# Tangshitao/Semi-supervised-Adaptive-Distillation

Hardware: AMD Instinct MI355X
Metric: images/sec (student+teacher fwd + student bwd) R50-FPN distill, 1/2/4/8 MI355X (higher is better)
Workload: dtype f32

## Files before the change

include/ssad_kernels.h:

```cpp
#ifndef SSAD_KERNELS_H_
#define SSAD_KERNELS_H_

#include <stddef.h>
#include <stdint.h>

#ifdef __cplusplus
extern "C" {
#endif

#define SSAD_API __attribute__((visibility("default")))

#define SSAD_E_BADARG (-1)
#define SSAD_E_WORKSPACE (-2)
#define SSAD_MAX_LEVELS 8
#define SSAD_MAX_CONV_PROBLEMS 24
#define SSAD_MAX_POWSUM_INPUTS 8

typedef void* ssad_stream_t;


typedef struct {
  float gamma;
  float alpha;
  float beta;
// ... 128 lines not shown
  const float* x;
  float* y;
  const float* aux;
  int N, H, W;
  const float* packed;
  const float* bias;
} ssad_conv_level;

SSAD_API size_t ssad_conv_packed_filter_floats(int M, int K);

SSAD_API int ssad_conv_pack_filter(
    const float* w, int Cout, int Cin, float* packed_fwd, float* packed_dgrad,
    ssad_stream_t stream);

#define SSAD_CONV_RELU 1
#define SSAD_CONV_MASK_AUX 2
#define SSAD_CONV_SIGMOID 4
#define SSAD_CONV_SPLIT_TAIL 8

SSAD_API int ssad_conv3x3_forward(
    const ssad_conv_level* levels_host, int n_levels, const float* packed,
    const float* bias, int Cout, int Cin, int flags, ssad_stream_t stream);

SSAD_API size_t ssad_conv_wino_filter_floats(int M, int K);
SSAD_API int ssad_conv_wino_pack_filter(
    const float* w, int Cout, int Cin, float* packed_fwd, float* packed_dgrad,
    ssad_stream_t stream);
SSAD_API int ssad_conv3x3_forward_wino(
    const ssad_conv_level* levels_host, int n_levels, const float* packed,
    const float* bias, int Cout, int Cin, int flags, ssad_stream_t stream);
SSAD_API int ssad_conv3x3_forward_wino_launches(const ssad_conv_level* levels_host, int n_levels);
SSAD_API int ssad_conv3x3_forward_wino_launches_for(const ssad_conv_level* levels_host, int n_levels, int Cout,
                                                    int Cin, int flags);
SSAD_API int ssad_conv_wino_split_tail(int on);
#define SSAD_MAX_PACK_ENTRIES 32
typedef struct ssad_pack_entry {
  const float* w;
  int Cout, Cin;
  float* packed_fwd;
  float* packed_dgrad;
} ssad_pack_entry;
SSAD_API int ssad_conv_wino_pack_filters(const ssad_pack_entry* entries_host, int n_entries,
                                         ssad_stream_t stream);

SSAD_API size_t ssad_conv_wino24_filter_floats(int M, int K);
SSAD_API int ssad_conv_wino24_pack_filters(const ssad_pack_entry* entries_host, int n_entries, ssad_stream_t stream);
SSAD_API int ssad_conv3x3_forward_wino24(
    const ssad_conv_level* levels_host, int n_levels, const float* packed,
    const float* bias, int Cout, int Cin, int flags, ssad_stream_t stream);

SSAD_API size_t ssad_conv_split_filter_floats(int M, int K);
SSAD_API int ssad_conv_split_pack_filters(const ssad_pack_entry* entries_host, int n_entries, ssad_stream_t stream);
SSAD_API size_t ssad_conv3x3_split_workspace_bytes(const ssad_conv_level* levels_host, int n_levels, int Cin);
SSAD_API int ssad_conv3x3_forward_split(
    const ssad_conv_level* levels_host, int n_levels, const float* packed,
    const float* bias, int Cout, int Cin, int flags, void* workspace, size_t workspace_bytes,
    const unsigned* amax_in, unsigned* amax_out, ssad_stream_t stream);

SSAD_API size_t ssad_conv3x3_wgrad_workspace_bytes(
    const ssad_conv_level* levels_host, int n_levels, int Cout, int Cin);

SSAD_API int ssad_conv3x3_wgrad(
    const ssad_conv_level* levels_host, int n_levels, float* dW, float* db,
    int Cout, int Cin, int accumulate, void* workspace, size_t workspace_bytes,
    ssad_stream_t stream);

SSAD_API size_t ssad_conv3x3_wgrad_split_workspace_bytes(
    const ssad_conv_level* levels_host, int n_levels, int Cout, int Cin);
SSAD_API int ssad_conv3x3_wgrad_split(
    const ssad_conv_level* levels_host, int n_levels, float* dW, float* db,
    int Cout, int Cin, int accumulate, void* workspace, size_t workspace_bytes,
    ssad_stream_t stream);
SSAD_API int ssad_conv3x3_wgrad_split_amax(
    const ssad_conv_level* levels_host, int n_levels, float* dW, float* db,
    int Cout, int Cin, int accumulate, void* workspace, size_t workspace_bytes,
    const unsigned* x_amax, const unsigned* dy_amax, ssad_stream_t stream);

SSAD_API int ssad_split_absmax_levels(const ssad_conv_level* levels_host, int n, int channels, int field,
                                      unsigned* words, ssad_stream_t stream);
SSAD_API int ssad_split_absmax(const float* x, long long n, unsigned* word, ssad_stream_t stream);


SSAD_API size_t ssad_retinanet_anchor_labels_workspace_bytes(
    int levels, int A, int k_min, const int* field_sizes_host, int N, int Gmax);
SSAD_API int ssad_retinanet_anchor_labels(
    const double* cell_anchors, int levels, int A, int k_min, const int* field_sizes_host,
    const int* crop_h_host, const int* crop_w_host, const float* gt_boxes,
    const int* gt_classes, const int* gt_counts, int N, int Gmax, int num_classes,
    float positive_overlap, float negative_overlap, int* const* labels_out_host,
    float* const* locs_out_host, float* const* targets_out_host, int capacity,
    int* counts_out, float* fg_bg_out, void* workspace, size_t workspace_bytes,
    ssad_stream_t stream);


#define SSAD_IMAGE_BLOBS_MAX_BATCH 64
typedef struct ssad_image_norm {
  float div, mean[3], std[3];
  float* out;
} ssad_image_norm;
SSAD_API size_t ssad_image_blobs_workspace_bytes(int N, int Hb, int Wb);
SSAD_API int ssad_image_blobs(
    const unsigned char* src, size_t src_bytes, const long long* offset_host, const int* h_host,
    const int* w_host, const int* out_h_host, const int* out_w_host, const double* scale_host,
    const int* flipped_host, int N, int Hb, int Wb, const ssad_image_norm* norms_host, int n_norms,
    void* workspace, size_t workspace_bytes, ssad_stream_t stream);

// ... 278 lines not shown
```

semi-supervised-adaptive-distillation_amd/csrc/kernels/conv3x3_split.hip:

```cpp
#include <hip/hip_fp16.h>
#include <hip/hip_runtime.h>
#include <stdint.h>
#include <stdlib.h>

#include "conv_internal.h"
#include "ssad_kernels.h"

#include "split_common.h"

namespace {

using namespace ssad_split;

constexpr int TS = 16;
constexpr int HS = TS + 2;
constexpr int CBC = 2;
constexpr int SLOTS = CBC * HS * HS;
constexpr int NLD = 3;
constexpr int STAGE = 4 * NLD * 64;
constexpr int AD = 9;
constexpr int NBUF = 3;
constexpr int MT = 128;
constexpr int HDR = 16;
static_assert(AD == 9 && NLD == 3, "the counted waits below are written for these");

#ifndef SPLIT_ABLATE
#define SPLIT_ABLATE 0
#endif

#ifdef SPLIT_TIMELINE
__device__ unsigned long long g_split_dbg[64][8];
#define SDBG(itn, k) if (dbg_on && (itn) < 64) g_split_dbg[itn][k] = __builtin_readcyclecounter()
#else
#define SDBG(itn, k)
#endif

__host__ __device__ constexpr int cdiv(int a, int b) { return (a + b - 1) / b; }

struct FPackTable {
  ssad_pack_entry e[SSAD_MAX_PACK_ENTRIES];
};
__global__ void split_filter_zero_kernel(const FPackTable t) {
  const ssad_pack_entry& e = t.e[blockIdx.x];
  if (threadIdx.x < HDR) {
    if (e.packed_fwd) reinterpret_cast<unsigned*>(e.packed_fwd)[threadIdx.x] = 0u;
    if (e.packed_dgrad) reinterpret_cast<unsigned*>(e.packed_dgrad)[threadIdx.x] = 0u;
  }
}
__global__ __launch_bounds__(kThreads) void split_filter_amax_kernel(const FPackTable t) {
  const ssad_pack_entry& e = t.e[blockIdx.y];
  const long long n = (long long)e.Cout * e.Cin * 9;
  unsigned m = 0;
  for (long long i = (long long)blockIdx.x * kThreads + threadIdx.x; i < n; i += (long long)gridDim.x * kThreads) {
    const unsigned a = __float_as_uint(e.w[i]) & 0x7fffffffu;
    m = m > a ? m : a;
  }
  __shared__ unsigned red[kThreads / 64];
#pragma unroll
  for (int o = 32; o > 0; o >>= 1) {
    const unsigned other = (unsigned)__shfl_xor((int)m, o, 64);
    m = m > other ? m : other;
  }
  if ((threadIdx.x & 63) == 0) red[threadIdx.x >> 6] = m;
  __syncthreads();
  if (threadIdx.x == 0) {
    unsigned r = red[0];
    for (int w = 1; w < kThreads / 64; ++w) r = r > red[w] ? r : red[w];
    if (r) {
      if (e.packed_fwd) atomicMax(reinterpret_cast<unsigned*>(e.packed_fwd), r);
      if (e.packed_dgrad) atomicMax(reinterpret_cast<unsigned*>(e.packed_dgrad), r);
    }
  }
}
__global__ __launch_bounds__(kThreads) void split_filter_pack_kernel(const FPackTable t) {
  const ssad_pack_entry& e = t.e[blockIdx.y];
  const bool dg = blockIdx.z == 1;
  float* dst = dg ? e.packed_dgrad : e.packed_fwd;
  if (!dst) return;
  const int M = dg ? e.Cin : e.Cout, K = dg ? e.Cout : e.Cin;
  const int KB = (K + 7) >> 3;
  const long long slots = 9LL * KB * M;
  const float s = pow2f(15 - split_exponent(reinterpret_cast<const unsigned*>(dst)[0]));
  uint4* out = reinterpret_cast<uint4*>(dst + HDR);
  for (long long i = (long long)blockIdx.x * kThreads + threadIdx.x; i < slots; i += (long long)gridDim.x * kThreads) {
    const int m = (int)(i % M), kb = (int)((i / M) % KB), tap = (int)(i / ((long long)M * KB));
    float v[8];
#pragma unroll
    for (int j = 0; j < 8; ++j) {
      const int k = kb * 8 + j;
      v[j] = k >= K ? 0.0f : dg ? e.w[((long long)k * e.Cin + m) * 9 + (8 - tap)] : e.w[((long long)m * e.Cin + k) * 9 + tap];
    }
    half8 hi, lo;
    split8(v, s, hi, lo);
    out[i] = __builtin_bit_cast(uint4, hi);
    out[slots + i] = __builtin_bit_cast(uint4, lo);
  }
}

struct SLevels {
  const uint4* x[kMaxLv];
  float* y[kMaxLv];
  const float* aux[kMaxLv];
  const float* w[kMaxLv];
  const float* bias[kMaxLv];
  int N[kMaxLv], H[kMaxLv], W[kMaxLv];
  int tile0[kMaxLv + 1];
  const unsigned* amax;
  unsigned* amax_out;
  int n_levels, C, M, relu, sigmoid, mblocks, items;
};

template <bool MASKED>
__global__ __launch_bounds__(kThreads, 1) void conv3x3_split_kernel(const SLevels q) {
  __shared__ uint4 lds[NBUF * 2 * STAGE];
  __shared__ unsigned wg_max[kThreads / 64];
  const int tid = threadIdx.x, lane = tid & 63;
  const int wave = __builtin_amdgcn_readfirstlane(tid >> 6);
  const int wo = wave & 1, wp = wave >> 1;
  const int j = lane & 31, h = lane >> 5;
  const int C = q.C, M = q.M;
  const int CB = (C + 7) >> 3;
  const int nchunks = (CB + CBC - 1) / CBC;
  const unsigned w_lo_off = (unsigned)(9LL * CB * M * 16);
  const unsigned lds_base = (unsigned)(uintptr_t)(lds_ptr)lds;
  const int brow = wp * 8 + (j >> 4), bcol = (j & 16) ? ((j - 2) & 15) : j;
  const int bbase = (h * HS + brow) * HS + bcol;

  struct Item {
    int lv, n, y0, x0, ocb, H, W, N;
  };
  auto decode = [&](int it) {
    Item o;
    const int xcd = it & 7, seq = it >> 3;
    const int mb = seq % q.mblocks;
    int t = (seq / q.mblocks) * 8 + xcd;
    int lv = 0;
    for (int l = 1; l < q.n_levels; ++l)
      if (t >= q.tile0[l]) lv = l;
    o.lv = t < q.tile0[q.n_levels] ? lv : -1;
    o.N = q.N[lv]; o.H = q.H[lv]; o.W = q.W[lv];
    const int tiles_x = (o.W + TS - 1) / TS, tiles_y = (o.H + TS - 1) / TS;
    t -= q.tile0[lv];
    const int tx = t % tiles_x; t /= tiles_x;
    const int ty = t % tiles_y;
    o.n = t / tiles_y;
    o.y0 = ty * TS; o.x0 = tx * TS;
    o.ocb = mb * MT;
    return o;
  };
  ssad_dev::rsrc_words xrs = ssad_dev::uniform_rsrc_words(q.x[0], 0), wrs = xrs;
  unsigned dvo[NLD], avo[2], x_lo_off = 0;
  int dcb[NLD], plane16 = 0;
  auto bind = [&](const Item& I) {
    const long long plane = (long long)I.H * I.W;
    plane16 = (int)plane * 16;
    x_lo_off = (unsigned)((long long)I.N * CB * plane16);
    xrs = ssad_dev::uniform_rsrc_words(q.x[I.lv], 2u * x_lo_off);
    wrs = ssad_dev::uniform_rsrc_words(q.w[I.lv] + HDR, 2u * w_lo_off);
#pragma unroll
    for (int i = 0; i < NLD; ++i) {
      const int s = 64 * (wave + 4 * i) + lane;
      const int cbl = s / (HS * HS), r = s % (HS * HS);
      const int gy = I.y0 - 1 + r / HS, gx = I.x0 - 1 + r % HS;
      const bool ok = s < SLOTS && gy >= 0 && gy < I.H && gx >= 0 && gx < I.W;
      dcb[i] = cbl;
      dvo[i] = ok ? (unsigned)((((long long)I.n * CB + cbl) * plane + (long long)gy * I.W + gx) * 16) : kOob;
    }
#pragma unroll
    for (int i = 0; i < 2; ++i) {
      const int oc = I.ocb + wo * 64 + i * 32 + j;
      avo[i] = (unsigned)(h * M + (oc < M ? oc : M - 1)) * 16u;
    }
  };
  auto dma_piece = [&](int chunk, int buf, int i, bool real) {
    const unsigned vo = (real && !(SPLIT_ABLATE & 1) && chunk * CBC + dcb[i] < CB) ? dvo[i] : kOob;
    const int soff = __builtin_amdgcn_readfirstlane(real ? chunk * CBC * plane16 : 0);
    const unsigned dst = lds_base + (unsigned)((buf * 2 * STAGE + 64 * (wave + 4 * i)) * 16);
    dma16(xrs, dst, vo, soff);
    dma16(xrs, dst + STAGE * 16, vo, soff + (int)x_lo_off);
  };
  f32x4 ar[AD][4];
  auto ring_load1 = [&](f32x4& dst, int chunk, int tap, int k, bool real) {
    const int soff = __builtin_amdgcn_readfirstlane(real ? ((tap * CB + chunk * CBC) * M) * 16 + (k >> 1) * (int)w_lo_off : 0);
    const unsigned vo = (real && !(SPLIT_ABLATE & 2)) ? avo[k & 1] : kOob;
    asm volatile("s_nop 4\n\tbuffer_load_dwordx4 %0, %1, %2, %3 offen" : "=v"(dst) : "v"(vo), "s"(wrs), "s"(soff));
  };
  auto ring_load = [&](f32x4 (&dst)[4], int chunk, int tap, bool real) {
#pragma unroll
    for (int k = 0; k < 4; ++k) ring_load1(dst[k], chunk, tap, k, real);
  };
  auto ring_landed = [&]() {
    asm volatile("s_waitcnt vmcnt(0)" ::: "memory");
#pragma unroll
    for (int a = 0; a < AD; ++a) asm volatile("" : "+v"(ar[a][0]), "+v"(ar[a][1]), "+v"(ar[a][2]), "+v"(ar[a][3]));
  };
  int gbuf = 0;
  auto prologue = [&]() {
    int b1 = gbuf + 1; if (b1 >= NBUF) b1 -= NBUF;
#pragma unroll
    for (int i = 0; i < NLD; ++i) dma_piece(0, gbuf, i, true);
#pragma unroll
    for (int i = 0; i < NLD; ++i) dma_piece(1, b1, i, nchunks > 1);
#pragma unroll
    for (int a = 0; a < AD; ++a) ring_load(ar[a], 0, a, true);
  };

  const int G = (int)gridDim.x;
  int it = (int)blockIdx.x;
  Item cur = decode(it);
  while (it < q.items && cur.lv < 0) { it += G; if (it < q.items) cur = decode(it); }
  if (it >= q.items) return;
  bind(cur);
  prologue();
  ring_landed();
  __builtin_amdgcn_s_barrier();

#ifdef SPLIT_TIMELINE
  const bool dbg_on = blockIdx.x == 5 && tid == 0;
  int itn = 0;
#endif
  while (true) {
    SDBG(itn, 0);
    float16v acc[2][4];
    {
      float zero;
      asm volatile("v_mov_b32 %0, 0" : "=v"(zero));
#pragma unroll
      for (int i = 0; i < 2; ++i)
#pragma unroll
        for (int tt = 0; tt < 4; ++tt)
#pragma unroll
          for (int r = 0; r < 16; ++r) acc[i][tt][r] = zero;
    }

    int buf = gbuf;
    for (int c = 0; c < nchunks; ++c) {
      const bool more = c + 1 < nchunks, more2 = c + 2 < nchunks;
      int buf2 = buf + 2; if (buf2 >= NBUF) buf2 -= NBUF;
      const uint4* tile_hi = lds + buf * 2 * STAGE;
      const uint4* tile_lo = tile_hi + STAGE;
      half8 bh[4], bl[4];
      auto read_b = [&](const uint4* tile, int tap, half8 (&bb)[4]) {
        const int dy = tap / 3, dx = tap % 3;
#pragma unroll
        for (int tt = 0; tt < 4; ++tt) bb[tt] = __builtin_bit_cast(half8, tile[bbase + (2 * tt + dy) * HS + dx]);
      };
      read_b(tile_hi, 0, bh);
      read_b(tile_lo, 0, bl);
#pragma unroll
      for (int tap = 0; tap < 9; ++tap) {
        f32x4 (&a)[4] = ar[tap];
        switch (tap) {
          case 0: asm volatile("s_waitcnt vmcnt(38)" : "+v"(a[0]), "+v"(a[1]), "+v"(a[2]), "+v"(a[3])); break;
          case 7: case 8: asm volatile("s_waitcnt vmcnt(34)" : "+v"(a[0]), "+v"(a[1]), "+v"(a[2]), "+v"(a[3])); break;
          default: asm volatile("s_waitcnt vmcnt(36)" : "+v"(a[0]), "+v"(a[1]), "+v"(a[2]), "+v"(a[3])); break;
        }
        const half8 ah0 = __builtin_bit_cast(half8, a[0]), ah1 = __builtin_bit_cast(half8, a[1]);
        const half8 al0 = __builtin_bit_cast(half8, a[2]), al1 = __builtin_bit_cast(half8, a[3]);
        __builtin_amdgcn_sched_barrier(0);
#pragma unroll
        for (int tt = 0; tt < 4; ++tt) {
          acc[0][tt] = __builtin_amdgcn_mfma_f32_32x32x16_f16(ah0, bh[tt], acc[0][tt], 0, 0, 0);
          acc[1][tt] = __builtin_amdgcn_mfma_f32_32x32x16_f16(ah1, bh[tt], acc[1][tt], 0, 0, 0);
          if (tap >= 1) {
            __builtin_amdgcn_sched_barrier(0);
            if (tt < 2) ring_load1(ar[tap - 1][tt], c + 1, tap - 1, tt, more);
            if (tt == 2 && tap - 1 >= 9 - NLD) dma_piece(c + 2, buf2, tap - 1 - (9 - NLD), more2);
            __builtin_amdgcn_sched_barrier(0);
          }
        }
        __builtin_amdgcn_sched_barrier(0);
        if (!(SPLIT_ABLATE & 4)) {
#pragma unroll
          for (int tt = 0; tt < 4; ++tt) {
            acc[0][tt] = __builtin_amdgcn_mfma_f32_32x32x16_f16(al0, bh[tt], acc[0][tt], 0, 0, 0);
            acc[1][tt] = __builtin_amdgcn_mfma_f32_32x32x16_f16(al1, bh[tt], acc[1][tt], 0, 0, 0);
          }
        }
        __builtin_amdgcn_sched_barrier(0);
        if (tap + 1 < 9) read_b(tile_hi, tap + 1, bh);
        __builtin_amdgcn_sched_barrier(0);
#pragma unroll
        for (int tt = 0; tt < 4; ++tt) {
          if (!(SPLIT_ABLATE & 4)) {
            acc[0][tt] = __builtin_amdgcn_mfma_f32_32x32x16_f16(ah0, bl[tt], acc[0][tt], 0, 0, 0);
            acc[1][tt] = __builtin_amdgcn_mfma_f32_32x32x16_f16(ah1, bl[tt], acc[1][tt], 0, 0, 0);
          }
          __builtin_amdgcn_sched_barrier(0);
          if (tt < 2) ring_load1(a[2 + tt], c + 1, tap, 2 + tt, more);
          __builtin_amdgcn_sched_barrier(0);
        }
        if (tap + 1 < 9) read_b(tile_lo, tap + 1, bl);
        if (tap == 8) {
          ring_load1(a[0], c + 1, 8, 0, more);
          ring_load1(a[1], c + 1, 8, 1, more);
          dma_piece(c + 2, buf2, NLD - 1, more2);
        }
        __builtin_amdgcn_sched_barrier(0);
      }
      asm volatile("s_waitcnt vmcnt(42) lgkmcnt(0)" ::: "memory");
      __builtin_amdgcn_s_barrier();
      if (++buf == NBUF) buf = 0;
    }
    SDBG(itn, 1);
    gbuf = buf;
    ring_landed();

    const Item done = cur;
    int nit = it + G;
    Item nxt = done;
    while (nit < q.items) { nxt = decode(nit); if (nxt.lv >= 0) break; nit += G; }
    const bool have_next = nit < q.items;
    const long long plane = (long long)done.H * done.W;
    const int oc_w = done.ocb + wo * 64;
    unsigned pvo[4];
#pragma unroll
    for (int tt = 0; tt < 4; ++tt) {
      const int gy = done.y0 + wp * 8 + 2 * tt + (j >> 4), gx = done.x0 + bcol;
      const bool okp = gy < done.H && gx < done.W;
      const long long pix = (long long)gy * done.W + gx;
      pvo[tt] = okp ? (unsigned)((((long long)done.n * M + 4 * h) * plane + pix) * 4) : kOob;
    }
    SDBG(itn, 2);
#if !(SPLIT_ABLATE & 32)
    if (have_next) {
      bind(nxt);
      prologue();
    }
#endif
    SDBG(itn, 3);

    {
      const int lv = done.lv;
      const int e2 = split_exponent(q.amax[lv]) + split_exponent(reinterpret_cast<const unsigned*>(q.w[lv])[0]) - 30;
      const bool one_scale = e2 >= -126 && e2 <= 127;
      const float sc1 = one_scale ? pow2f(e2) : pow2f(split_exponent(q.amax[lv]) - 15);
      const float sc2 = one_scale ? 1.0f : pow2f(split_exponent(reinterpret_cast<const unsigned*>(q.w[lv])[0]) - 15);
      const unsigned ybytes = (unsigned)((long long)done.N * M * plane * 4);
      const __amdgpu_buffer_rsrc_t yrs = uniform_rsrc(q.y[lv], ybytes);
      const __amdgpu_buffer_rsrc_t mrs = uniform_rsrc(MASKED ? (const void*)q.aux[lv] : (const void*)q.y[lv], ybytes);
      const float* bias = q.bias[lv];
      const __amdgpu_buffer_rsrc_t brs = uniform_rsrc(bias ? (const void*)bias : (const void*)q.y[lv],
                                                      bias ? (unsigned)M * 4u : 0u);
      const bool relu = q.relu, sigm = q.sigmoid;
      const bool ragged = (M & 7) != 0;
      const bool want_max = q.amax_out != nullptr;
      const int plane4 = (int)plane * 4;
      unsigned vmax = 0;
#pragma unroll
      for (int i = 0; i < 2; ++i) {
        const int oc0 = oc_w + i * 32;
        float4 bq[4];
#pragma unroll
        for (int g = 0; g < 4; ++g)
          bq[g] = __builtin_bit_cast(float4, __builtin_amdgcn_raw_buffer_load_b128(brs, (unsigned)h * 16u, (oc0 + 8 * g) * 4, 0));
#pragma unroll
        for (int tt = 0; tt < 4; ++tt) {
          float mk[16];
          if (MASKED) {
#pragma unroll
            for (int r = 0; r < 16; ++r) {
              const int ch = oc0 + 8 * (r >> 2) + (r & 3);
              const unsigned vo = (!ragged || ch + 4 * h < M) ? pvo[tt] : kOob;
              mk[r] = __builtin_bit_cast(float, __builtin_amdgcn_raw_buffer_load_b32(mrs, vo, ch * plane4, 0));
            }
          }
#pragma unroll
          for (int g = 0; g < 4; ++g) {
            if (oc0 + 8 * g >= M) continue;
#pragma unroll
            for (int e = 0; e < 4; ++e) {
              float v = one_scale ? fmaf(acc[i][tt][4 * g + e], sc1, bq[g][e]) : acc[i][tt][4 * g + e] * sc1 * sc2 + bq[g][e];
              if (relu) v = fmaxf(v, 0.0f);
              if (sigm) v = 1.0f / (1.0f + expf(-v));
              if (MASKED) v = mk[4 * g + e] > 0.0f ? v : 0.0f;
              const unsigned vo = (!ragged || oc0 + 8 * g + 4 * h + e < M) ? pvo[tt] : kOob;
              if (want_max) {
                const unsigned av = __float_as_uint(v) & 0x7fffffffu;
                vmax = (vo != kOob && av > vmax) ? av : vmax;
              }
              __builtin_amdgcn_raw_buffer_store_b32(__builtin_bit_cast(unsigned, v), yrs, vo, (oc0 + 8 * g + e) * plane4, 0);
            }
          }
        }
      }
      if (q.amax_out) {
#pragma unroll
        for (int o = 32; o > 0; o >>= 1) {
          const unsigned other = (unsigned)__shfl_xor((int)vmax, o, 64);
          vmax = vmax > other ? vmax : other;
        }
        if (lane == 0) wg_max[wave] = vmax;
      }
    }
#if SPLIT_ABLATE & 32
    if (have_next) {
      asm volatile("s_waitcnt vmcnt(0)" ::: "memory");
      bind(nxt);
      prologue();
    }
#endif
    if (!have_next) {
      if (q.amax_out) {
        __builtin_amdgcn_s_barrier();
        if (tid == 0) {
          unsigned m = wg_max[0];
          for (int w = 1; w < kThreads / 64; ++w) m = m > wg_max[w] ? m : wg_max[w];
          if (m) atomicMax(q.amax_out + done.lv, m);
        }
      }
      asm volatile("s_waitcnt vmcnt(0)" ::: "memory");
      return;
    }
    SDBG(itn, 4);
    ring_landed();
    SDBG(itn, 5);
    __builtin_amdgcn_s_barrier();
    SDBG(itn, 6);
#ifdef SPLIT_TIMELINE
    ++itn;
#endif
    if (q.amax_out && tid == 0) {
      unsigned m = wg_max[0];
      for (int w = 1; w < kThreads / 64; ++w) m = m > wg_max[w] ? m : wg_max[w];
      if (m) atomicMax(q.amax_out + done.lv, m);
    }
    it = nit;
    cur = nxt;
  }
}

struct Plan {
  size_t amax_bytes, total_bytes;
  size_t plane_off[kMaxLv];
  long long slots[kMaxLv];
};
int make_plan(const ssad_conv_level* lv, int n_levels, int Cin, Plan* p) {
  if (!lv || n_levels < 1 || n_levels > kMaxLv || Cin <= 0) return SSAD_E_BADARG;
  const int CB = (Cin + 7) >> 3;
  p->amax_bytes = 256;
  size_t off = p->amax_bytes;
  for (int l = 0; l < n_levels; ++l) {
    if (lv[l].N < 0 || lv[l].H < 0 || lv[l].W < 0) return SSAD_E_BADARG;
    const long long slots = (long long)lv[l].N * CB * lv[l].H * lv[l].W;
    if (slots * 32 >= (1LL << 32)) return SSAD_E_BADARG;
    p->slots[l] = slots;
    p->plane_off[l] = off;
    off += (size_t)slots * 32;
    off = (off + 255) & ~(size_t)255;
  }
  p->total_bytes = off;
  return 0;
}

}

#ifdef SPLIT_TIMELINE
extern "C" __attribute__((visibility("default"))) int ssad_split_dbg_read(void* host) {
  return (int)hipMemcpyFromSymbol(host, HIP_SYMBOL(g_split_dbg), sizeof(g_split_dbg));
}
#endif

extern "C" {

size_t ssad_conv_split_filter_floats(int M, int K) {
  return (size_t)HDR + 2 * (size_t)9 * ((K + 7) >> 3) * M * 4 + 64;
}

int ssad_conv_split_pack_filters(const ssad_pack_entry* entries_host, int n_entries, ssad_stream_t stream) {
  if (n_entries < 0 || (n_entries > 0 && !entries_host)) return SSAD_E_BADARG;
  for (int base = 0; base < n_entries; base += SSAD_MAX_PACK_ENTRIES) {
    const int cnt = n_entries - base < SSAD_MAX_PACK_ENTRIES ? n_entries - base : SSAD_MAX_PACK_ENTRIES;
    FPackTable t;
    long long smax = 0;
    bool any_dgrad = false;
    for (int i = 0; i < cnt; ++i) {
      const ssad_pack_entry& e = entries_host[base + i];
      if (e.Cout <= 0 || e.Cin <= 0 || !e.w || (!e.packed_fwd && !e.packed_dgrad)) return SSAD_E_BADARG;
      t.e[i] = e;
      const long long sf = 9LL * ((e.Cin + 7) >> 3) * e.Cout, sd = 9LL * ((e.Cout + 7) >> 3) * e.Cin;
      smax = sf > smax ? sf : smax;
      if (e.packed_dgrad) { smax = sd > smax ? sd : smax; any_dgrad = true; }
    }
    for (int i = cnt; i < SSAD_MAX_PACK_ENTRIES; ++i) t.e[i] = ssad_pack_entry{};
    hipLaunchKernelGGL(split_filter_zero_kernel, dim3((unsigned)cnt), dim3(64), 0, (hipStream_t)stream, t);
    hipLaunchKernelGGL(split_filter_amax_kernel, dim3(64u, (unsigned)cnt), dim3(kThreads), 0, (hipStream_t)stream, t);
    long long bx = (smax + kThreads - 1) / kThreads;
    if (bx > 512) bx = 512;
    hipLaunchKernelGGL(split_filter_pack_kernel, dim3((unsigned)bx, (unsigned)cnt, any_dgrad ? 2u : 1u), dim3(kThreads), 0,
                       (hipStream_t)stream, t);
  }
  return (int)hipGetLastError();
}

size_t ssad_conv3x3_split_workspace_bytes(const ssad_conv_level* lv, int n_levels, int Cin) {
  Plan p;
  if (make_plan(lv, n_levels, Cin, &p)) return 0;
  return p.total_bytes;
}

int ssad_conv3x3_forward_split(const ssad_conv_level* lv, int n_levels, const float* packed, const float* bias,
                               int Cout, int Cin, int flags, void* workspace, size_t workspace_bytes,
                               const unsigned* amax_in, unsigned* amax_out, ssad_stream_t stream_) {
  hipStream_t stream = (hipStream_t)stream_;
  Plan p;
  const int rc = make_plan(lv, n_levels, Cin, &p);
  if (rc) return rc;
  if (Cout <= 0) return SSAD_E_BADARG;
  if ((flags & SSAD_CONV_MASK_AUX) && (flags & SSAD_CONV_SIGMOID)) return SSAD_E_BADARG;
  if (!workspace || workspace_bytes < p.total_bytes) return SSAD_E_WORKSPACE;
  AmaxTable at;
  ActTable pt;
  SLevels q;
  at.count = pt.count = 0;
  at.amax = (unsigned*)workspace;
  pt.amax = q.amax = (const unsigned*)workspace;
  q.amax_out = amax_out;
  pt.C = Cin;
  int nl = 0, ablocks = 0, pblocks = 0, tiles = 0;
  for (int l = 0; l < n_levels; ++l) {
    const float* pk = lv[l].packed ? lv[l].packed : packed;
    if (!pk) return SSAD_E_BADARG;
    if ((flags & SSAD_CONV_MASK_AUX) && !lv[l].aux) return SSAD_E_BADARG;
    const long long px = (long long)lv[l].N * lv[l].H * lv[l].W;
    if (px * (Cin > Cout ? Cin : Cout) >= (1LL << 29)) return SSAD_E_BADARG;
    if (px == 0) continue;
    const long long n = px * Cin;
    at.x[nl] = pt.x[nl] = lv[l].x;
    at.n[nl] = n;
    at.block_start[nl] = ablocks;
    long long nb = (n / 4 + kThreads * 32 - 1) / (kThreads * 32);
    ablocks += (int)(nb < 1 ? 1 : nb > 512 ? 512 : nb);
    pt.planes[nl] = (uint4*)((char*)workspace + p.plane_off[l]);
    pt.N[nl] = lv[l].N;
    pt.plane[nl] = (long long)lv[l].H * lv[l].W;
    pt.block_start[nl] = pblocks;
    int same = -1;
    for (int j = 0; j < nl && same < 0; ++j)
      if (at.x[j] == lv[l].x && q.N[j] == lv[l].N && q.H[j] == lv[l].H && q.W[j] == lv[l].W) same = j;
    if (same >= 0) pt.planes[nl] = (uint4*)q.x[same];
    else pblocks += (int)((p.slots[l] + kThreads - 1) / kThreads);
    q.x[nl] = (const uint4*)pt.planes[nl];
    q.y[nl] = lv[l].y;
    q.aux[nl] = lv[l].aux;
    q.w[nl] = pk;
    q.bias[nl] = lv[l].packed ? lv[l].bias : bias;
    q.N[nl] = lv[l].N; q.H[nl] = lv[l].H; q.W[nl] = lv[l].W;
    q.tile0[nl] = tiles;
    tiles += lv[l].N * cdiv(lv[l].H, TS) * cdiv(lv[l].W, TS);
    ++nl;
  }
  if (nl == 0) return 0;
  at.block_start[nl] = ablocks;
  pt.block_start[nl] = pblocks;
  q.tile0[nl] = tiles;
  at.count = pt.count = q.n_levels = nl;
  for (int l = nl; l < kMaxLv; ++l) {
    at.x[l] = pt.x[l] = nullptr; at.n[l] = 0; pt.planes[l] = nullptr; pt.N[l] = 0; pt.plane[l] = 0;
    q.x[l] = nullptr; q.y[l] = nullptr; q.aux[l] = nullptr; q.w[l] = nullptr; q.bias[l] = nullptr;
    q.N[l] = q.H[l] = q.W[l] = 0;
    if (l > nl) { at.block_start[l] = ablocks; pt.block_start[l] = pblocks; q.tile0[l] = tiles; }
  }
  q.C = Cin; q.M = Cout;
  q.relu = (flags & SSAD_CONV_RELU) ? 1 : 0;
  q.sigmoid = (flags & SSAD_CONV_SIGMOID) ? 1 : 0;
  q.mblocks = cdiv(Cout, MT);
  if ((amax_in || amax_out) && nl != n_levels) return SSAD_E_BADARG;
  if (amax_in) {
    pt.amax = q.amax = amax_in;
  } else {
    (void)hipMemsetAsync(workspace, 0, p.amax_bytes, stream);
    hipLaunchKernelGGL(split_absmax_kernel, dim3((unsigned)ablocks), dim3(kThreads), 0, stream, at);
  }
  hipLaunchKernelGGL(split_pack_act_kernel, dim3((unsigned)pblocks), dim3(kThreads), 0, stream, pt);
  q.items = cdiv(tiles, 8) * 8 * q.mblocks;
  const int cus = ssad_cu_count();
  const unsigned grid = (unsigned)(q.items < cus ? q.items : cus);
  if (flags & SSAD_CONV_MASK_AUX)
    hipLaunchKernelGGL((conv3x3_split_kernel<true>), dim3(grid), dim3(kThreads), 0, stream, q);
  else
    hipLaunchKernelGGL((conv3x3_split_kernel<false>), dim3(grid), dim3(kThreads), 0, stream, q);
  return (int)hipGetLastError();
}

int ssad_split_absmax_levels(const ssad_conv_level* lv, int n, int channels, int field, unsigned* words,
                             ssad_stream_t stream_) {
  if (!lv || !words || n < 1 || n > kMaxLv || channels <= 0) return SSAD_E_BADARG;
  AmaxTable at;
  int blocks = 0;
  for (int l = 0; l < kMaxLv; ++l) {
    at.x[l] = nullptr; at.n[l] = 0; at.block_start[l] = blocks;
    if (l >= n) continue;
    const long long cnt = (long long)lv[l].N * lv[l].H * lv[l].W * channels;
    at.x[l] = field ? lv[l].aux : lv[l].x;
    at.n[l] = cnt;
    if (cnt && !at.x[l]) return SSAD_E_BADARG;
    long long nb = (cnt / 4 + kThreads * 32 - 1) / (kThreads * 32);
    blocks += (int)(nb < 1 ? 1 : nb > 512 ? 512 : nb);
  }
  at.block_start[kMaxLv] = blocks;
  at.count = n;
  at.amax = words;
  hipLaunchKernelGGL(split_absmax_kernel, dim3((unsigned)blocks), dim3(kThreads), 0, (hipStream_t)stream_, at);
  return (int)hipGetLastError();
}

}
```

semi-supervised-adaptive-distillation_amd/kernels.py:

```python
import ctypes as C
import os

import torch

_HERE = os.path.dirname(os.path.abspath(__file__))
LIB_NAME = "libcaffe2_detectron_ops_hip.so"
LIB_PATH = os.path.join(_HERE, LIB_NAME)

MAX_LEVELS = 8
CONV_RELU = 1
CONV_MASK_AUX = 2
CONV_SIGMOID = 4
CONV_SPLIT_TAIL = 8


class KernelError(RuntimeError):
    pass


class DistillParams(C.Structure):
    _fields_ = [("gamma", C.c_float), ("alpha", C.c_float), ("beta", C.c_float),
                ("num_classes", C.c_int), ("ignored_label", C.c_int),
                ("scale", C.c_float)]

# ... 137 lines not shown
    L.ssad_fill.argtypes = [vp, f32, i64, vp]
    L.ssad_pow_sum_workspace_bytes.restype = sz
    L.ssad_pow_sum_workspace_bytes.argtypes = [i32]
    L.ssad_pow_sum.argtypes = [C.POINTER(vp), C.POINTER(i64), i32, f32, vp, vp, sz, vp]
    L.ssad_pow_sum_prezeroed.argtypes = L.ssad_pow_sum.argtypes
    L.ssad_relu.argtypes = [vp, vp, i64, vp]
    L.ssad_relu_grad.argtypes = [vp, vp, vp, i64, vp]
    L.ssad_sigmoid.argtypes = [vp, vp, i64, vp]
    L.ssad_sum_n.argtypes = [C.POINTER(vp), i32, vp, i64, vp]
    L.ssad_scale.argtypes = [vp, vp, f32, i64, vp]
    L.ssad_affine_channel.argtypes = [vp, vp, vp, vp, vp, i32, i32, i32, i32, vp]
    L.ssad_upsample_nearest.argtypes = [vp, vp, vp, i32, i32, i32, i32, i32, vp]
    L.ssad_upsample_nearest_grad.argtypes = [vp, vp, i32, i32, i32, i32, i32, vp]
    L.ssad_max_pool3x3s2_bias_relu.argtypes = [vp, vp, i32, i32, i32, i32, i32, vp, vp]
    L.ssad_relu_grad_rowsum.argtypes = [vp, vp, vp, vp, i32, i32, i32, vp]
    L.ssad_conv1x1_bias_act.argtypes = [vp, vp, vp, vp, vp, i32, i32, i32, i32, i32, vp]
    L.ssad_conv1x1_bias_act2.argtypes = [vp, i32, vp, i32, vp, vp, vp, vp, i32, i32, i32, i32, vp]
    L.ssad_f16_pack_activations.argtypes = [vp, i32, i32, i32, i32, f32, vp, vp]
    L.ssad_f16_unpack_activations.argtypes = [vp, i32, i32, i32, i32, f32, vp, vp]
    L.ssad_f16_filter_halves.restype = sz
    L.ssad_f16_filter_halves.argtypes = [i32, i32]
    L.ssad_f16_pack_filter.argtypes = [vp, i32, i32, vp, vp, vp]
    L.ssad_conv3x3_forward_f16.argtypes = [vp, vp, vp, vp, i32, i32, i32, i32, i32, i32, vp, vp]
    L.ssad_conv3x3_forward_f16_levels.argtypes = [C.POINTER(F16Level), i32, vp, vp, i32, i32, i32, vp]
    L.ssad_conv3x3_wgrad_f16_workspace_bytes.restype = sz
    L.ssad_conv3x3_wgrad_f16_workspace_bytes.argtypes = [i32, i32, i32, i32, i32]
    L.ssad_conv3x3_wgrad_f16.argtypes = [vp, vp, i32, i32, i32, i32, i32, i32, f32, vp, vp, vp, sz, vp]
    L.ssad_conv3x3_wgrad_f16_levels_workspace_bytes.restype = sz
    L.ssad_conv3x3_wgrad_f16_levels_workspace_bytes.argtypes = [C.POINTER(F16WgradLevel), i32, i32, i32]
    L.ssad_conv3x3_wgrad_f16_levels.argtypes = [C.POINTER(F16WgradLevel), i32, i32, i32, i32, f32, vp, vp,
                                                vp, sz, vp]
    L.ssad_momentum_sgd_update.argtypes = [vp, vp, vp, vp, f32, f32, i32, i64, vp]
    L.ssad_momentum_sgd_flat.argtypes = [vp, vp, vp, vp, f32, f32, C.POINTER(SgdSegment), i32, vp, vp]
    L.ssad_check_finite.argtypes = [vp, i64, vp, vp]
    L.ssad_loss_scale_update.argtypes = [vp, vp, f32, f32, i32, f32, f32, vp]
    L.ssad_conv_wino_pack_filters.argtypes = [C.POINTER(PackEntry), i32, vp]
    L.ssad_conv_packed_filter_floats.restype = sz
    L.ssad_conv_packed_filter_floats.argtypes = [i32, i32]
    L.ssad_conv_pack_filter.argtypes = [vp, i32, i32, vp, vp, vp]
    L.ssad_conv3x3_forward.argtypes = [C.POINTER(ConvLevel), i32, vp, vp, i32, i32, i32, vp]
    L.ssad_conv_wino_filter_floats.restype = sz
    L.ssad_conv_wino_filter_floats.argtypes = [i32, i32]
    L.ssad_conv_wino_pack_filter.argtypes = [vp, i32, i32, vp, vp, vp]
    L.ssad_conv3x3_forward_wino.argtypes = [C.POINTER(ConvLevel), i32, vp, vp, i32, i32, i32, vp]
    L.ssad_conv3x3_forward_wino24.argtypes = [C.POINTER(ConvLevel), i32, vp, vp, i32, i32, i32, vp]
    L.ssad_conv_wino24_filter_floats.restype = sz
    L.ssad_conv_wino24_filter_floats.argtypes = [i32, i32]
    L.ssad_conv_wino24_pack_filters.argtypes = [C.POINTER(PackEntry), i32, vp]
    L.ssad_conv_split_filter_floats.restype = sz
    L.ssad_conv_split_filter_floats.argtypes = [i32, i32]
    L.ssad_conv_split_pack_filters.argtypes = [C.POINTER(PackEntry), i32, vp]
    L.ssad_conv3x3_split_workspace_bytes.restype = sz
    L.ssad_conv3x3_split_workspace_bytes.argtypes = [C.POINTER(ConvLevel), i32, i32]
    L.ssad_conv3x3_forward_split.argtypes = [C.POINTER(ConvLevel), i32, vp, vp, i32, i32, i32, vp, sz, vp, vp, vp]
    L.ssad_conv3x3_forward_wino_launches.argtypes = [C.POINTER(ConvLevel), i32]
    L.ssad_conv3x3_forward_wino_launches_for.argtypes = [C.POINTER(ConvLevel), i32, i32, i32, i32]
    L.ssad_conv_wino_split_tail.argtypes = [i32]
    L.ssad_conv3x3_wgrad_workspace_bytes.restype = sz
    L.ssad_conv3x3_wgrad_workspace_bytes.argtypes = [C.POINTER(ConvLevel), i32, i32, i32]
    L.ssad_conv3x3_wgrad.argtypes = [C.POINTER(ConvLevel), i32, vp, vp, i32, i32, i32, vp, sz, vp]
    L.ssad_conv3x3_wgrad_split_workspace_bytes.restype = sz
    L.ssad_conv3x3_wgrad_split_workspace_bytes.argtypes = [C.POINTER(ConvLevel), i32, i32, i32]
    L.ssad_conv3x3_wgrad_split.argtypes = [C.POINTER(ConvLevel), i32, vp, vp, i32, i32, i32, vp, sz, vp]
    L.ssad_conv1x1_gemm.argtypes = [C.POINTER(GemmConv), vp]
    L.ssad_conv1x1_gemm_split_workspace_bytes.restype = sz
    L.ssad_conv1x1_gemm_split_workspace_bytes.argtypes = [C.POINTER(GemmConv)]
    L.ssad_conv1x1_gemm_split.argtypes = [C.POINTER(GemmConv), vp, sz, vp]
    L.ssad_transpose_filter.argtypes = [vp, i32, i32, i32, vp, vp]
    L.ssad_conv1x1_wgrad_workspace_bytes.restype = sz
    L.ssad_conv1x1_wgrad_workspace_bytes.argtypes = [i32, i32, i32, i32]
    L.ssad_conv1x1_wgrad.argtypes = [vp, vp, i32, i32, i32, i32, vp, i32, vp, sz, vp]
    L.ssad_gemm_split_filter_floats.restype = sz
    L.ssad_gemm_split_filter_floats.argtypes = [i32, i32]
    L.ssad_gemm_split_pack_filters.argtypes = [C.POINTER(GemmPackEntry), i32, vp]
    L.ssad_conv1x1_gemm_split_amax.argtypes = [vp, vp, vp, vp, vp, sz, vp]
    L.ssad_split_absmax.argtypes = [vp, C.c_longlong, vp, vp]
    L.ssad_split_absmax_levels.argtypes = [C.POINTER(ConvLevel), i32, i32, i32, vp, vp]
    L.ssad_conv3x3_wgrad_split_amax.argtypes = [C.POINTER(ConvLevel), i32, vp, vp, i32, i32, i32, vp, sz, vp, vp, vp]
    L.ssad_conv1x1_wgrad_split_amax.argtypes = [vp, vp, i32, i32, i32, i32, vp, i32, vp, sz, vp, vp, vp]
    L.ssad_conv1x1_wgrad_split_workspace_bytes.restype = sz
    L.ssad_conv1x1_wgrad_split_workspace_bytes.argtypes = [i32, i32, i32, i32]
    L.ssad_conv1x1_wgrad_split.argtypes = [vp, vp, i32, i32, i32, i32, vp, i32, vp, sz, vp]
    L.ssad_subsample.argtypes = [vp, i32, i32, i32, i32, i32, vp, vp]
    L.ssad_subsample_grad.argtypes = [vp, i32, i32, i32, i32, i32, i32, vp, vp]
    L.ssad_conv_implicit_gemm.argtypes = [C.POINTER(GemmConv), i32, i32, i32, i32, i32, i32, vp]
    L.ssad_transpose_filters.argtypes = [C.POINTER(TransposeEntry), i32, vp]
    L.ssad_f16_pack_filters.argtypes = [C.POINTER(F16PackEntry), i32, vp]
    L.ssad_conv_implicit_gemm_workspace_bytes.restype = sz
    L.ssad_conv_implicit_gemm_workspace_bytes.argtypes = [i32] * 8
    L.ssad_conv_implicit_gemm_ws.argtypes = [C.POINTER(GemmConv), i32, i32, i32, i32, i32, i32, vp, sz, vp]
    L.ssad_conv_kxk_wgrad_workspace_bytes.restype = sz
    L.ssad_conv_kxk_wgrad_workspace_bytes.argtypes = [i32] * 8
    L.ssad_conv_kxk_wgrad.argtypes = [vp, vp, i32, i32, i32, i32, i32, i32, i32, i32, vp, i32, vp, sz, vp]
    L.ssad_conv_kxk_dgrad_workspace_bytes.restype = sz
    L.ssad_conv_kxk_dgrad_workspace_bytes.argtypes = [i32] * 8
    L.ssad_conv_kxk_dgrad.argtypes = [vp, vp, i32, i32, i32, i32, i32, i32, i32, i32, vp, vp, i32, vp, sz, vp]
    L.ssad_grouped_conv3x3_forward.argtypes = [vp, vp, vp, i32, i32, i32, i32, i32, i32, i32, vp, vp]
    L.ssad_grouped_conv3x3_filter_floats.argtypes = [i32, i32]
    L.ssad_grouped_conv3x3_filter_floats.restype = C.c_longlong
    L.ssad_grouped_conv3x3_pack_filter.argtypes = [vp, i32, i32, vp, vp]
    L.ssad_conv1x1_f16.argtypes = [C.POINTER(PwF16), vp]
    L.ssad_pw_f16_filter_halves.restype = sz
    L.ssad_pw_f16_filter_halves.argtypes = [i32, i32]
    L.ssad_pw_f16_pack_filter.argtypes = [vp, i32, i32, vp, vp, vp]
    L.ssad_conv1x1_wgrad_f16_workspace_bytes.restype = sz
    L.ssad_conv1x1_wgrad_f16_workspace_bytes.argtypes = [i32, i32, i32, i32, i32]
# ... 467 lines not shown
                     device="cuda") if want_dgrad else None
    _check(L.ssad_conv_wino_pack_filter(_ptr(w), Cout, Cin, _ptr(pf), _ptr(pd), _stream()),
           "conv_wino_pack_filter")
    return pf, pd


def conv_wino24_pack_filter(w, want_dgrad=False):
    L = lib()
    _f32c(w, "filter")
    Cout, Cin, kh, kw = w.shape
    if (kh, kw) != (3, 3):
        raise KernelError("only 3x3 filters")
    pf = torch.empty(L.ssad_conv_wino24_filter_floats(Cout, Cin), dtype=torch.float32, device="cuda")
    pd = torch.empty(L.ssad_conv_wino24_filter_floats(Cin, Cout), dtype=torch.float32,
                     device="cuda") if want_dgrad else None
    tab = (PackEntry * 1)(PackEntry(w.data_ptr(), Cout, Cin, pf.data_ptr(), pd.data_ptr() if want_dgrad else 0))
    _check(L.ssad_conv_wino24_pack_filters(tab, 1, _stream()), "conv_wino24_pack_filters")
    return (pf, pd) if want_dgrad else pf


def conv_split_pack_filter(w, want_dgrad=False):
    L = lib()
    _f32c(w, "filter")
    Cout, Cin, kh, kw = w.shape
    if (kh, kw) != (3, 3):
        raise KernelError("only 3x3 filters")
    pf = torch.empty(L.ssad_conv_split_filter_floats(Cout, Cin), dtype=torch.float32, device="cuda")
    pd = torch.empty(L.ssad_conv_split_filter_floats(Cin, Cout), dtype=torch.float32,
                     device="cuda") if want_dgrad else None
    tab = (PackEntry * 1)(PackEntry(w.data_ptr(), Cout, Cin, pf.data_ptr(), pd.data_ptr() if want_dgrad else 0))
    _check(L.ssad_conv_split_pack_filters(tab, 1, _stream()), "conv_split_pack_filters")
    return (pf, pd) if want_dgrad else pf


def conv3x3_forward_split(xs, packed, bias, Cout, *, relu=False, sigmoid=False, out=None, mask_by=None, workspace=None,
                          amax_in=None, amax_out=None):
    L = lib()
    for x in xs:
        _f32c(x, "conv input")
    Cin = xs[0].shape[1]
    ys = out if out is not None else [
        torch.empty((x.shape[0], Cout, x.shape[2], x.shape[3]), dtype=torch.float32, device="cuda") for x in xs]
    flags = (CONV_RELU if relu else 0) | (CONV_SIGMOID if sigmoid else 0) | (CONV_MASK_AUX if mask_by is not None else 0)
    arr = _conv_levels(xs, ys, mask_by)
    need = L.ssad_conv3x3_split_workspace_bytes(arr, len(xs), Cin)
    if workspace is None or workspace.numel() < need:
        workspace = torch.empty(max(need, 16), dtype=torch.uint8, device="cuda")
    _check(L.ssad_conv3x3_forward_split(arr, len(xs), _ptr(packed), _ptr(bias), Cout, Cin, flags, _ptr(workspace),
                                        workspace.numel(), _ptr(amax_in), _ptr(amax_out), _stream()),
           "conv3x3_forward_split")
    return ys


def conv3x3_forward_wino24(xs, packed, bias, Cout, *, relu=False, sigmoid=False, out=None, mask_by=None):
    L = lib()
    for x in xs:
        _f32c(x, "conv input")
    Cin = xs[0].shape[1]
    ys = out if out is not None else [
        torch.empty((x.shape[0], Cout, x.shape[2], x.shape[3]), dtype=torch.float32, device="cuda") for x in xs]
    flags = (CONV_RELU if relu else 0) | (CONV_SIGMOID if sigmoid else 0) | (CONV_MASK_AUX if mask_by is not None else 0)
    arr = _conv_levels(xs, ys, mask_by)
    _check(L.ssad_conv3x3_forward_wino24(arr, len(xs), _ptr(packed), _ptr(bias), Cout, Cin, flags, _stream()),
           "conv3x3_forward_wino24")
    return ys


def _conv_levels(xs, ys, auxs, packs=None, biases=None):
    n = len(xs)
    arr = (ConvLevel * n)()
    for i in range(n):
        N, _, H, W = xs[i].shape
        arr[i] = ConvLevel(xs[i].data_ptr(),
                           ys[i].data_ptr() if ys is not None and ys[i] is not None else 0,
                           auxs[i].data_ptr() if auxs is not None and auxs[i] is not None else 0,
                           N, H, W,
                           packs[i].data_ptr() if packs is not None else 0,
                           biases[i].data_ptr() if biases is not None and biases[i] is not None else 0)
    return arr


def conv3x3_forward(xs, packed, bias, Cout, *, relu=False, sigmoid=False, mask_by=None,
                    out=None, wino=False):
    L = lib()
    for x in xs:
        _f32c(x, "conv input")
    Cin = xs[0].shape[1]
    ys = out if out is not None else [
        torch.empty((x.shape[0], Cout, x.shape[2], x.shape[3]), dtype=torch.float32,
                    device="cuda") for x in xs]
    flags = ((CONV_RELU if relu else 0) | (CONV_MASK_AUX if mask_by is not None else 0)
             | (CONV_SIGMOID if sigmoid else 0))
    arr = _conv_levels(xs, ys, mask_by)
    fn = L.ssad_conv3x3_forward_wino if wino else L.ssad_conv3x3_forward
    _check(fn(arr, len(xs), _ptr(packed), _ptr(bias), Cout, Cin, flags, _stream()),
           "conv3x3_forward")
    return ys


def conv3x3_forward_multi(problems, Cout, *, relu=False, sigmoid=False, wino=False):
    L = lib()
    xs, ys, auxs, packs, biases = [], [], [], [], []
    for p in problems:
        n = len(p["xs"])
        xs += list(p["xs"]); ys += list(p["out"])
        auxs += list(p["mask_by"]) if p.get("mask_by") is not None else [None] * n
# ... 359 lines not shown
```

Baseline: 240.4.

## Pack two half-height tiles per work item in split conv3x3 for odd-row levels

For FPN levels whose height in 8-row half-tiles is odd, each 16x16 work item now covers two independent 8-row half tiles, possibly from different rows or images. Each wave pair computes one half with its own halo rows in the LDS stage. This avoids computing and loading a mostly padded bottom tile when the height is not a multiple of 16. It adds more complex decode and halo addressing, plus extra lgkmcnt waits before barriers. It is enabled by default through an environment variable.

```diff
diff --git a/include/ssad_kernels.h b/include/ssad_kernels.h
--- a/include/ssad_kernels.h
+++ b/include/ssad_kernels.h
@@ -204,6 +204,7 @@
 SSAD_API size_t ssad_conv_split_filter_floats(int M, int K);
 SSAD_API int ssad_conv_split_pack_filters(const ssad_pack_entry* entries_host, int n_entries, ssad_stream_t stream);
 SSAD_API size_t ssad_conv3x3_split_workspace_bytes(const ssad_conv_level* levels_host, int n_levels, int Cin);
+SSAD_API int ssad_conv3x3_split_items(const ssad_conv_level* levels_host, int n_levels, int Cout);
 SSAD_API int ssad_conv3x3_forward_split(
     const ssad_conv_level* levels_host, int n_levels, const float* packed,
     const float* bias, int Cout, int Cin, int flags, void* workspace, size_t workspace_bytes,
diff --git a/semi-supervised-adaptive-distillation_amd/csrc/kernels/conv3x3_split.hip b/semi-supervised-adaptive-distillation_amd/csrc/kernels/conv3x3_split.hip
--- a/semi-supervised-adaptive-distillation_amd/csrc/kernels/conv3x3_split.hip
+++ b/semi-supervised-adaptive-distillation_amd/csrc/kernels/conv3x3_split.hip
@@ -13,9 +13,11 @@
 using namespace ssad_split;
 
 constexpr int TS = 16;
+constexpr int HT = TS / 2;
 constexpr int HS = TS + 2;
+constexpr int HR = 2 * (HT + 2);
 constexpr int CBC = 2;
-constexpr int SLOTS = CBC * HS * HS;
+constexpr int SLOTS = CBC * HR * HS;
 constexpr int NLD = 3;
 constexpr int STAGE = 4 * NLD * 64;
 constexpr int AD = 9;
@@ -23,6 +25,7 @@
 constexpr int MT = 128;
 constexpr int HDR = 16;
 static_assert(AD == 9 && NLD == 3, "the counted waits below are written for these");
+static_assert(SLOTS <= STAGE, "a plane's halo blocks fit the stage");
 
 #ifndef SPLIT_ABLATE
 #define SPLIT_ABLATE 0
@@ -104,6 +107,7 @@
   const float* w[kMaxLv];
   const float* bias[kMaxLv];
   int N[kMaxLv], H[kMaxLv], W[kMaxLv];
+  int half[kMaxLv];
   int tile0[kMaxLv + 1];
   const unsigned* amax;
   unsigned* amax_out;
@@ -123,11 +127,24 @@
   const int nchunks = (CB + CBC - 1) / CBC;
   const unsigned w_lo_off = (unsigned)(9LL * CB * M * 16);
   const unsigned lds_base = (unsigned)(uintptr_t)(lds_ptr)lds;
-  const int brow = wp * 8 + (j >> 4), bcol = (j & 16) ? ((j - 2) & 15) : j;
-  const int bbase = (h * HS + brow) * HS + bcol;
+  const int bcol = (j & 16) ? ((j - 2) & 15) : j;
+  const int bbase0 = (h * HR + (j >> 4)) * HS + bcol;
 
   struct Item {
-    int lv, n, y0, x0, ocb, H, W, N;
+    int lv, ocb, H, W, N, half;
+    int n0, y0, x0, n1, y1, x1;
+  };
+  struct Own {
+    int lv, ocb;
+    int n, y0, x0;
+    int boff;
+  };
+  auto own = [&](const Item& I) {
+    Own o;
+    o.lv = I.lv; o.ocb = I.ocb;
+    o.n = wp ? I.n1 : I.n0; o.y0 = wp ? I.y1 : I.y0; o.x0 = wp ? I.x1 : I.x0;
+    o.boff = wp * (I.half ? HT + 2 : HT) * HS;
+    return o;
   };
   auto decode = [&](int it) {
     Item o;
@@ -139,12 +156,23 @@
       if (t >= q.tile0[l]) lv = l;
     o.lv = t < q.tile0[q.n_levels] ? lv : -1;
     o.N = q.N[lv]; o.H = q.H[lv]; o.W = q.W[lv];
-    const int tiles_x = (o.W + TS - 1) / TS, tiles_y = (o.H + TS - 1) / TS;
+    o.half = q.half[lv];
+    const int tiles_x = (o.W + TS - 1) / TS, tiles_y = o.half ? (o.H + HT - 1) / HT : (o.H + TS - 1) / TS;
     t -= q.tile0[lv];
-    const int tx = t % tiles_x; t /= tiles_x;
-    const int ty = t % tiles_y;
-    o.n = t / tiles_y;
-    o.y0 = ty * TS; o.x0 = tx * TS;
+    if (o.half) t *= 2;
+    int tx = t % tiles_x; t /= tiles_x;
+    int ty = t % tiles_y;
+    int n = t / tiles_y;
+    o.n0 = n; o.x0 = tx * TS;
+    if (o.half) {
+      o.y0 = ty * HT;
+      if (++tx == tiles_x) { tx = 0; if (++ty == tiles_y) { ty = 0; ++n; } }
+      const bool any = n < o.N;
+      o.n1 = any ? n : 0; o.y1 = any ? ty * HT : o.H + HT; o.x1 = tx * TS;
+    } else {
+      o.y0 = ty * TS;
+      o.n1 = n; o.y1 = o.y0 + HT; o.x1 = o.x0;
+    }
     o.ocb = mb * MT;
     return o;
   };
@@ -160,11 +188,13 @@
 #pragma unroll
     for (int i = 0; i < NLD; ++i) {
       const int s = 64 * (wave + 4 * i) + lane;
-      const int cbl = s / (HS * HS), r = s % (HS * HS);
-      const int gy = I.y0 - 1 + r / HS, gx = I.x0 - 1 + r % HS;
-      const bool ok = s < SLOTS && gy >= 0 && gy < I.H && gx >= 0 && gx < I.W;
+      const int cbl = s / (HR * HS), r = s % (HR * HS);
+      const int row = r / HS, col = r % HS;
+      const bool p = I.half && row >= HT + 2;
+      const int gy = (p ? I.y1 - (HT + 2) : I.y0) - 1 + row, gx = (p ? I.x1 : I.x0) - 1 + col;
+      const bool ok = s < SLOTS && (I.half || row < HS) && gy >= 0 && gy < I.H && gx >= 0 && gx < I.W;
       dcb[i] = cbl;
-      dvo[i] = ok ? (unsigned)((((long long)I.n * CB + cbl) * plane + (long long)gy * I.W + gx) * 16) : kOob;
+      dvo[i] = ok ? (unsigned)((((long long)(p ? I.n1 : I.n0) * CB + cbl) * plane + (long long)gy * I.W + gx) * 16) : kOob;
     }
 #pragma unroll
     for (int i = 0; i < 2; ++i) {
@@ -207,10 +237,11 @@
 
   const int G = (int)gridDim.x;
   int it = (int)blockIdx.x;
-  Item cur = decode(it);
-  while (it < q.items && cur.lv < 0) { it += G; if (it < q.items) cur = decode(it); }
+  Item first = decode(it);
+  while (it < q.items && first.lv < 0) { it += G; if (it < q.items) first = decode(it); }
   if (it >= q.items) return;
-  bind(cur);
+  bind(first);
+  Own cur = own(first);
   prologue();
   ring_landed();
   __builtin_amdgcn_s_barrier();
@@ -234,6 +265,7 @@
     }
 
     int buf = gbuf;
+    const int bbase = bbase0 + cur.boff;
     for (int c = 0; c < nchunks; ++c) {
       const bool more = c + 1 < nchunks, more2 = c + 2 < nchunks;
       int buf2 = buf + 2; if (buf2 >= NBUF) buf2 -= NBUF;
@@ -306,19 +338,21 @@
     gbuf = buf;
     ring_landed();
 
-    const Item done = cur;
+    const Own done = cur;
     int nit = it + G;
-    Item nxt = done;
+    Item nxt{};
     while (nit < q.items) { nxt = decode(nit); if (nxt.lv >= 0) break; nit += G; }
     const bool have_next = nit < q.items;
-    const long long plane = (long long)done.H * done.W;
+    const Own nown = own(nxt);
+    const int doneH = q.H[done.lv], doneW = q.W[done.lv];
+    const long long plane = (long long)doneH * doneW;
     const int oc_w = done.ocb + wo * 64;
     unsigned pvo[4];
 #pragma unroll
     for (int tt = 0; tt < 4; ++tt) {
-      const int gy = done.y0 + wp * 8 + 2 * tt + (j >> 4), gx = done.x0 + bcol;
-      const bool okp = gy < done.H && gx < done.W;
-      const long long pix = (long long)gy * done.W + gx;
+      const int gy = done.y0 + 2 * tt + (j >> 4), gx = done.x0 + bcol;
+      const bool okp = gy < doneH && gx < doneW;
+      const long long pix = (long long)gy * doneW + gx;
       pvo[tt] = okp ? (unsigned)((((long long)done.n * M + 4 * h) * plane + pix) * 4) : kOob;
     }
     SDBG(itn, 2);
@@ -336,7 +370,7 @@
       const bool one_scale = e2 >= -126 && e2 <= 127;
       const float sc1 = one_scale ? pow2f(e2) : pow2f(split_exponent(q.amax[lv]) - 15);
       const float sc2 = one_scale ? 1.0f : pow2f(split_exponent(reinterpret_cast<const unsigned*>(q.w[lv])[0]) - 15);
-      const unsigned ybytes = (unsigned)((long long)done.N * M * plane * 4);
+      const unsigned ybytes = (unsigned)((long long)q.N[lv] * M * plane * 4);
       const __amdgpu_buffer_rsrc_t yrs = uniform_rsrc(q.y[lv], ybytes);
       const __amdgpu_buffer_rsrc_t mrs = uniform_rsrc(MASKED ? (const void*)q.aux[lv] : (const void*)q.y[lv], ybytes);
       const float* bias = q.bias[lv];
@@ -402,6 +436,7 @@
 #endif
     if (!have_next) {
       if (q.amax_out) {
+        asm volatile("s_waitcnt lgkmcnt(0)" ::: "memory");
         __builtin_amdgcn_s_barrier();
         if (tid == 0) {
           unsigned m = wg_max[0];
@@ -415,6 +450,7 @@
     SDBG(itn, 4);
     ring_landed();
     SDBG(itn, 5);
+    asm volatile("s_waitcnt lgkmcnt(0)" ::: "memory");
     __builtin_amdgcn_s_barrier();
     SDBG(itn, 6);
 #ifdef SPLIT_TIMELINE
@@ -426,7 +462,7 @@
       if (m) atomicMax(q.amax_out + done.lv, m);
     }
     it = nit;
-    cur = nxt;
+    cur = nown;
   }
 }
 
@@ -453,6 +489,15 @@
   return 0;
 }
 
+bool half_tiles_enabled() {
+  const char* e = getenv("SSAD_SPLIT_HALF_TILES");
+  return !(e && *e) || atoi(e) != 0;
+}
+bool level_half_mode(const ssad_conv_level& l, bool enabled) { return enabled && (cdiv(l.H, HT) & 1); }
+int level_tiles(const ssad_conv_level& l, bool half) {
+  return half ? cdiv(l.N * cdiv(l.H, HT) * cdiv(l.W, TS), 2) : l.N * cdiv(l.H, TS) * cdiv(l.W, TS);
+}
+
 }
 
 #ifdef SPLIT_TIMELINE
@@ -497,6 +542,18 @@
   Plan p;
   if (make_plan(lv, n_levels, Cin, &p)) return 0;
   return p.total_bytes;
+}
+
+int ssad_conv3x3_split_items(const ssad_conv_level* lv, int n_levels, int Cout) {
+  if (!lv || n_levels < 1 || n_levels > kMaxLv || Cout <= 0) return SSAD_E_BADARG;
+  const bool halves = half_tiles_enabled();
+  long long tiles = 0;
+  for (int l = 0; l < n_levels; ++l) {
+    if (lv[l].N < 0 || lv[l].H < 0 || lv[l].W < 0) return SSAD_E_BADARG;
+    if ((long long)lv[l].N * lv[l].H * lv[l].W * Cout >= (1LL << 29)) return SSAD_E_BADARG;
+    tiles += level_tiles(lv[l], level_half_mode(lv[l], halves));
+  }
+  return (int)(tiles * cdiv(Cout, MT));
 }
 
 int ssad_conv3x3_forward_split(const ssad_conv_level* lv, int n_levels, const float* packed, const float* bias,
@@ -518,6 +575,7 @@
   q.amax_out = amax_out;
   pt.C = Cin;
   int nl = 0, ablocks = 0, pblocks = 0, tiles = 0;
+  const bool halves = half_tiles_enabled();
   for (int l = 0; l < n_levels; ++l) {
     const float* pk = lv[l].packed ? lv[l].packed : packed;
     if (!pk) return SSAD_E_BADARG;
@@ -546,8 +604,9 @@
     q.w[nl] = pk;
     q.bias[nl] = lv[l].packed ? lv[l].bias : bias;
     q.N[nl] = lv[l].N; q.H[nl] = lv[l].H; q.W[nl] = lv[l].W;
+    q.half[nl] = level_half_mode(lv[l], halves) ? 1 : 0;
     q.tile0[nl] = tiles;
-    tiles += lv[l].N * cdiv(lv[l].H, TS) * cdiv(lv[l].W, TS);
+    tiles += level_tiles(lv[l], q.half[nl] != 0);
     ++nl;
   }
   if (nl == 0) return 0;
@@ -558,7 +617,7 @@
   for (int l = nl; l < kMaxLv; ++l) {
     at.x[l] = pt.x[l] = nullptr; at.n[l] = 0; pt.planes[l] = nullptr; pt.N[l] = 0; pt.plane[l] = 0;
     q.x[l] = nullptr; q.y[l] = nullptr; q.aux[l] = nullptr; q.w[l] = nullptr; q.bias[l] = nullptr;
-    q.N[l] = q.H[l] = q.W[l] = 0;
+    q.N[l] = q.H[l] = q.W[l] = q.half[l] = 0;
     if (l > nl) { at.block_start[l] = ablocks; pt.block_start[l] = pblocks; q.tile0[l] = tiles; }
   }
   q.C = Cin; q.M = Cout;
diff --git a/semi-supervised-adaptive-distillation_amd/kernels.py b/semi-supervised-adaptive-distillation_amd/kernels.py
--- a/semi-supervised-adaptive-distillation_amd/kernels.py
+++ b/semi-supervised-adaptive-distillation_amd/kernels.py
@@ -213,6 +213,7 @@
     L.ssad_conv_split_pack_filters.argtypes = [C.POINTER(PackEntry), i32, vp]
     L.ssad_conv3x3_split_workspace_bytes.restype = sz
     L.ssad_conv3x3_split_workspace_bytes.argtypes = [C.POINTER(ConvLevel), i32, i32]
+    L.ssad_conv3x3_split_items.argtypes = [C.POINTER(ConvLevel), i32, i32]
     L.ssad_conv3x3_forward_split.argtypes = [C.POINTER(ConvLevel), i32, vp, vp, i32, i32, i32, vp, sz, vp, vp, vp]
     L.ssad_conv3x3_forward_wino_launches.argtypes = [C.POINTER(ConvLevel), i32]
     L.ssad_conv3x3_forward_wino_launches_for.argtypes = [C.POINTER(ConvLevel), i32, i32, i32, i32]
@@ -786,6 +787,15 @@
     return ys
 
 
+def conv3x3_split_items(shapes, Cout):
+    arr = (ConvLevel * len(shapes))()
+    for i, (N, H, W) in enumerate(shapes):
+        arr[i] = ConvLevel(0, 0, 0, N, H, W, 0, 0)
+    n = lib().ssad_conv3x3_split_items(arr, len(shapes), Cout)
+    _check(min(n, 0), "conv3x3_split_items")
+    return n
+
+
 def conv3x3_forward_wino24(xs, packed, bias, Cout, *, relu=False, sigmoid=False, out=None, mask_by=None):
     L = lib()
     for x in xs:
```

New measurement: 247.0 (median of 6 runs). 1.03x the previous value.
